# nnnagle/vq-vae

Measured on AMD Instinct MI355X. Metric: tiles/sec, higher is better.
Workload: dtype bf16

## Files before the change

### vq-vae_amd/csrc/enc_fused.hip

```cpp
#include "frl_common.hpp"
#include "frl_host.hpp"
#include "frl_pack.hpp"
#include "frl_reduce.hpp"

typedef bf16 TT;
typedef bf16x8 frag8;
#define EF_C0 64
#define EF_C1 128
#define EF_C2 64
#define EF_G 8
#define EF_NW 8
#define EF_NTH (64 * EF_NW)
#define EF_W1_FRAGS (8 * 2 * 64)
#define EF_W2_FRAGS (4 * 4 * 64)
#define EF_W2T_FRAGS (8 * 2 * 64)
#define EF_SLAB 384

template <int CTRL> __device__ __forceinline__ float ef_dpp(float v) {
  return __builtin_bit_cast(float, __builtin_amdgcn_update_dpp(0, __builtin_bit_cast(int, v), CTRL, 0xf, 0xf, true));
}
__device__ __forceinline__ float ef_row_sum(float v) {
  v += ef_dpp<0xB1>(v);
  v += ef_dpp<0x4E>(v);
  v += ef_dpp<0x124>(v);
// ... 187 lines not shown
    }
    bf16x8* zo = reinterpret_cast<bf16x8*>(zb + (int64_t)(t * 16 + px) * EF_C2 + 16 * kc);
    zo[0] = o0;
    zo[1] = o1;
    xt = xn;
  }
}

template <int NCH>
__device__ __forceinline__ void ef_channel_totals(const float (&p0)[NCH], const float (&p1)[NCH], float* __restrict__ part, float* __restrict__ chan,
                                                  float* __restrict__ out0, float* __restrict__ out1, int tid) {
  constexpr int C = 4 * NCH;
  const int lane = tid & 63, wave = tid >> 6, px = lane & 15, kc = lane >> 4;
#pragma unroll
  for (int j = 0; j < NCH; ++j) {
    const float a = ef_row_sum(p0[j]), q = ef_row_sum(p1[j]);
    if (px == 0) { part[(wave * 2 + 0) * C + NCH * kc + j] = a; part[(wave * 2 + 1) * C + NCH * kc + j] = q; }
  }
  __syncthreads();
  for (int i = tid; i < 2 * C; i += EF_NTH) {
    const int which = i / C, c = i % C;
    float s = 0.f;
    for (int w = 0; w < EF_NW; ++w) s += part[(w * 2 + which) * C + c];
    chan[which * C + c] = s;
    (which == 0 ? out0 : out1)[c] = s;
  }
  __syncthreads();
}

#define EF_PA 72
#define EF_PB 136
#define EF_OFF_TA (EF_OFF_TAB + EF_T_END * 4)
#define EF_OFF_TB (EF_OFF_TA + 128 * EF_PA * 2)
#define EF_LDS_BWD (EF_OFF_TB + 128 * EF_PB * 2)
#define EF_SLAB2 (EF_C2 * EF_C1 + EF_C1 * EF_C0 + EF_SLAB)

__device__ __forceinline__ bf16x8 ef_tr_frag(const TT* tile, int pitch, int pix0, int ch0, int r16) {
  const TT* a0 = tile + (pix0 + (r16 >> 2)) * pitch + ch0 + 4 * (r16 & 3);
  const bf16x4 lo = __builtin_amdgcn_ds_read_tr16_b64_v4bf16((bf16x4 __attribute__((address_space(3)))*)(a0));
  const bf16x4 hi = __builtin_amdgcn_ds_read_tr16_b64_v4bf16((bf16x4 __attribute__((address_space(3)))*)(a0 + 4 * pitch));
  return bf16x8{lo[0], lo[1], lo[2], lo[3], hi[0], hi[1], hi[2], hi[3]};
}
template <int NF>
__device__ __forceinline__ void ef_tile_put(TT* tile, int pitch, int prow, int kc, const LQTile<TT, NF>& t) {
  bf16x8* p = reinterpret_cast<bf16x8*>(tile + prow * pitch + NF * 8 * kc);
#pragma unroll
  for (int s = 0; s < NF; ++s) p[s] = t.f[s];
}

__global__ __launch_bounds__(EF_NTH) void enc2_bwd_kernel(const TT* __restrict__ X, const TT* __restrict__ DZ, const frag8* __restrict__ Wpk,
                                                          const float* __restrict__ g1, const float* __restrict__ b1,
                                                          const float* __restrict__ g2, const float* __restrict__ b2,
                                                          const float* __restrict__ stats, float* __restrict__ slab, int HW) {
  extern __shared__ __attribute__((aligned(16))) char smem[];
  const frag8* w1 = reinterpret_cast<const frag8*>(smem);
  const frag8* w2 = reinterpret_cast<const frag8*>(smem + EF_OFF_W2);
  const frag8* w2t = reinterpret_cast<const frag8*>(smem + EF_OFF_W2T);
  float* tab = reinterpret_cast<float*>(smem + EF_OFF_TAB);
  float* chan = tab + EF_T_CH;
  float* part = chan + 4 * 128;
  TT* tA = reinterpret_cast<TT*>(smem + EF_OFF_TA);
  TT* tB = reinterpret_cast<TT*>(smem + EF_OFF_TB);
  const int tid = threadIdx.x, lane = tid & 63, wave = tid >> 6, px = lane & 15, kc = lane >> 4;
  const int b = blockIdx.x;
  const TT* xb = X + (int64_t)b * HW * EF_C0;
  const TT* dzb = DZ + (int64_t)b * HW * EF_C2;
  float* my = slab + (int64_t)b * EF_SLAB2;
  float* myg = my + EF_C2 * EF_C1 + EF_C1 * EF_C0;
  copy_frags_lds<TT>(reinterpret_cast<frag8*>(smem), Wpk, EF_W1_FRAGS + EF_W2_FRAGS + EF_W2T_FRAGS, tid, EF_NTH);
  if (tid < 32) tab[EF_T_ST1 + tid] = stats[(int64_t)b * 32 + tid];
  __syncthreads();
  for (int c = tid; c < EF_C1 + EF_C2; c += EF_NTH) {
    if (c < EF_C1) {
      const float a = tab[EF_T_ST1 + 8 + c / 16] * g1[c];
      tab[EF_T_A1 + c] = a;
      tab[EF_T_O1 + c] = fmaf(-tab[EF_T_ST1 + c / 16], a, b1[c]);
    } else {
      const int c2 = c - EF_C1;
      const float a = tab[EF_T_ST2 + 8 + c2 / 8] * g2[c2];
      tab[EF_T_A2 + c2] = a;
      tab[EF_T_O2 + c2] = fmaf(-tab[EF_T_ST2 + c2 / 8], a, b2[c2]);
    }
  }
  __syncthreads();
  const int ntile = HW >> 4;
  const int nround = (ntile + EF_NW - 1) / EF_NW;
  const float* a1q = tab + EF_T_A1 + 32 * kc;
  const float* o1q = tab + EF_T_O1 + 32 * kc;
  const float* a2q = tab + EF_T_A2 + 16 * kc;
  const float mu2[2] = {tab[EF_T_ST2 + 2 * kc], tab[EF_T_ST2 + 2 * kc + 1]}, rs2[2] = {tab[EF_T_ST2 + 8 + 2 * kc], tab[EF_T_ST2 + 8 + 2 * kc + 1]};
  const float mu1[2] = {tab[EF_T_ST1 + 2 * kc], tab[EF_T_ST1 + 2 * kc + 1]}, rs1[2] = {tab[EF_T_ST1 + 8 + 2 * kc], tab[EF_T_ST1 + 8 + 2 * kc + 1]};

  auto chain = [&](const LQTile<TT, 2>& xt, float (&y1)[32], LQTile<TT, 4>& ht, float (&y2)[16], int lw) {
    ef_conv1(y1, xt, w1, lw);
#pragma unroll
    for (int j = 0; j < 32; ++j) {
      float v = fmaf(y1[j], a1q[j], o1q[j]);
      v = v > 0.f ? v : 0.f;
      ht.f[j >> 3][j & 7] = (bf16)v;
    }
    ef_conv2(y2, ht, w2, lw);
  };

  {
    float p0[16], p1[16];
#pragma unroll
    for (int j = 0; j < 16; ++j) { p0[j] = 0.f; p1[j] = 0.f; }
    for (int t = wave; t < ntile; t += EF_NW) {
      int lw = lane;
      asm volatile("" : "+v"(lw));
      LQTile<TT, 2> xt, dt;
      lq_load<TT, 2>(xt, xb, t * 16 + px, EF_C0, kc, true);
      lq_load<TT, 2>(dt, dzb, t * 16 + px, EF_C2, kc, true);
      float y1[32], y2[16];
      LQTile<TT, 4> ht;
      chain(xt, y1, ht, y2, lw);
#pragma unroll
      for (int j = 0; j < 16; ++j) {
        const float d = (float)dt.f[j >> 3][j & 7];
        const float xh = (y2[j] - mu2[j >> 3]) * rs2[j >> 3];
        p0[j] += d;
        p1[j] = fmaf(d, xh, p1[j]);
      }
    }
    ef_channel_totals<16>(p0, p1, part, chan, myg, myg + 64, tid);
  }
  float e2[2], f2[2];
  {
    const float inv_n = 1.f / ((float)(EF_C2 / EF_G) * (float)HW);
#pragma unroll
    for (int g = 0; g < 2; ++g) {
      float S1 = 0.f, S2 = 0.f;
      for (int c = (2 * kc + g) * 8; c < (2 * kc + g + 1) * 8; ++c) { S1 = fmaf(g2[c], chan[c], S1); S2 = fmaf(g2[c], chan[64 + c], S2); }
      e2[g] = -rs2[g] * rs2[g] * S2 * inv_n;
      f2[g] = -rs2[g] * S1 * inv_n - e2[g] * mu2[g];
    }
  }
  __syncthreads();

  auto back2 = [&](const LQTile<TT, 2>& dt, const float (&y1)[32], const float (&y2)[16], LQTile<TT, 2>& gt, float (&d1)[32], int lw) {
#pragma unroll
    for (int j = 0; j < 16; ++j) {
      const float d = (float)dt.f[j >> 3][j & 7];
      gt.f[j >> 3][j & 7] = (bf16)fmaf(a2q[j], d, fmaf(e2[j >> 3], y2[j], f2[j >> 3]));
    }
#pragma unroll
    for (int m = 0; m < 8; ++m) {
      f32x4 a = f32x4{0.f, 0.f, 0.f, 0.f};
#pragma unroll
      for (int s = 0; s < 2; ++s) a = mfma16(w2t[(m * 2 + s) * 64 + lw], gt.f[s], a);
#pragma unroll
      for (int r = 0; r < 4; ++r) {
        const int j = 4 * m + r;
        float v = ef_r(a[r]);
        if (!(fmaf(y1[j], a1q[j], o1q[j]) > 0.f)) v = 0.f;
        d1[j] = v;
      }
    }
  };

  const int ob2 = wave & 3, ig2 = wave >> 2;
  {
    f32x4 acc2[4];
#pragma unroll
    for (int i = 0; i < 4; ++i) acc2[i] = f32x4{0.f, 0.f, 0.f, 0.f};
    float p0[32], p1[32];
#pragma unroll
    for (int j = 0; j < 32; ++j) { p0[j] = 0.f; p1[j] = 0.f; }
    for (int r = 0; r < nround; ++r) {
      const int t = r * EF_NW + wave;
      const bool valid = t < ntile;
      int lw = lane;
      asm volatile("" : "+v"(lw));
      LQTile<TT, 2> gt;
      LQTile<TT, 4> ht;
      if (valid) {
        LQTile<TT, 2> xt, dt;
        lq_load<TT, 2>(xt, xb, t * 16 + px, EF_C0, kc, true);
        lq_load<TT, 2>(dt, dzb, t * 16 + px, EF_C2, kc, true);
        float y1[32], y2[16], d1[32];
        chain(xt, y1, ht, y2, lw);
        back2(dt, y1, y2, gt, d1, lw);
#pragma unroll
        for (int j = 0; j < 32; ++j) {
          const float xh = (y1[j] - mu1[j >> 4]) * rs1[j >> 4];
          p0[j] += d1[j];
          p1[j] = fmaf(d1[j], xh, p1[j]);
        }
      } else {
#pragma unroll
        for (int s = 0; s < 2; ++s) gt.f[s] = frag8{};
#pragma unroll
        for (int s = 0; s < 4; ++s) ht.f[s] = frag8{};
      }
      ef_tile_put<2>(tA, EF_PA, wave * 16 + px, kc, gt);
      ef_tile_put<4>(tB, EF_PB, wave * 16 + px, kc, ht);
      __syncthreads();
#pragma unroll
      for (int ks = 0; ks < 4; ++ks) {
        const bf16x8 af = ef_tr_frag(tA, EF_PA, 32 * ks + 8 * kc, 16 * ob2, px);
#pragma unroll
        for (int i = 0; i < 4; ++i) acc2[i] = mfma16(af, ef_tr_frag(tB, EF_PB, 32 * ks + 8 * kc, 16 * (4 * ig2 + i), px), acc2[i]);
      }
      __syncthreads();
    }
#pragma unroll
    for (int i = 0; i < 4; ++i)
#pragma unroll
      for (int rr = 0; rr < 4; ++rr) my[(16 * ob2 + 4 * kc + rr) * EF_C1 + 16 * (4 * ig2 + i) + px] = acc2[i][rr];
    ef_channel_totals<32>(p0, p1, part, chan, myg + 128, myg + 256, tid);
  }
  float e1[2], f1[2];
  {
    const float inv_n = 1.f / ((float)(EF_C1 / EF_G) * (float)HW);
#pragma unroll
    for (int g = 0; g < 2; ++g) {
      float S1 = 0.f, S2 = 0.f;
      for (int c = (2 * kc + g) * 16; c < (2 * kc + g + 1) * 16; ++c) { S1 = fmaf(g1[c], chan[c], S1); S2 = fmaf(g1[c], chan[128 + c], S2); }
      e1[g] = -rs1[g] * rs1[g] * S2 * inv_n;
      f1[g] = -rs1[g] * S1 * inv_n - e1[g] * mu1[g];
    }
  }
  {
    f32x4 acc1[4];
#pragma unroll
    for (int i = 0; i < 4; ++i) acc1[i] = f32x4{0.f, 0.f, 0.f, 0.f};
    float* my1 = my + EF_C2 * EF_C1;
    for (int r = 0; r < nround; ++r) {
      const int t = r * EF_NW + wave;
      const bool valid = t < ntile;
      int lw = lane;
      asm volatile("" : "+v"(lw));
      LQTile<TT, 2> xt;
      LQTile<TT, 4> yt;
      if (valid) {
        LQTile<TT, 2> dt, gt;
        lq_load<TT, 2>(xt, xb, t * 16 + px, EF_C0, kc, true);
        lq_load<TT, 2>(dt, dzb, t * 16 + px, EF_C2, kc, true);
        float y1[32], y2[16], d1[32];
        LQTile<TT, 4> ht;
        chain(xt, y1, ht, y2, lw);
        back2(dt, y1, y2, gt, d1, lw);
#pragma unroll
        for (int j = 0; j < 32; ++j) yt.f[j >> 3][j & 7] = (bf16)fmaf(a1q[j], d1[j], fmaf(e1[j >> 4], y1[j], f1[j >> 4]));
      } else {
#pragma unroll
        for (int s = 0; s < 2; ++s) xt.f[s] = frag8{};
#pragma unroll
        for (int s = 0; s < 4; ++s) yt.f[s] = frag8{};
      }
      ef_tile_put<2>(tA, EF_PA, wave * 16 + px, kc, xt);
      ef_tile_put<4>(tB, EF_PB, wave * 16 + px, kc, yt);
      __syncthreads();
#pragma unroll
      for (int ks = 0; ks < 4; ++ks) {
        const bf16x8 af = ef_tr_frag(tB, EF_PB, 32 * ks + 8 * kc, 16 * wave, px);
#pragma unroll
        for (int i = 0; i < 4; ++i) acc1[i] = mfma16(af, ef_tr_frag(tA, EF_PA, 32 * ks + 8 * kc, 16 * i, px), acc1[i]);
      }
      __syncthreads();
    }
#pragma unroll
    for (int i = 0; i < 4; ++i)
#pragma unroll
      for (int rr = 0; rr < 4; ++rr) my1[(16 * wave + 4 * kc + rr) * EF_C0 + 16 * i + px] = acc1[i][rr];
  }
}


static const frag8* enc_packed(const float* w1, const float* w2, int bwd, frag8* ws_pk, hipStream_t st) {
  FrlPackJob jobs[3];
  size_t off = 0;
  jobs[0] = frl_pack_job_pw(w1, off, FRL_BF16, 2, EF_C1, EF_C0, 8, EF_C0, 1);
  off += (size_t)EF_W1_FRAGS * sizeof(frag8);
  jobs[1] = frl_pack_job_pw(w2, off, FRL_BF16, 4, EF_C2, EF_C1, 4, EF_C1, 1);
  off += (size_t)EF_W2_FRAGS * sizeof(frag8);
  int n = 2;
  if (bwd) {
    jobs[2] = frl_pack_job_pw(w2, off, FRL_BF16, 2, EF_C1, EF_C2, 8, 1, EF_C1);
    off += (size_t)EF_W2T_FRAGS * sizeof(frag8);
    n = 3;
  }
  bool hit = false;
  frag8* pk = ws_pk;
  if (void* img = frl_pack_cached(jobs, n, off, &hit)) pk = (frag8*)img;
  if (!hit) {
    FRL_LAUNCH((pack_weights_kernel<TT, 2>), dim3(4), dim3(256), 0, st, pk, w1, EF_C1, EF_C0, 8, (int64_t)EF_C0, (int64_t)1);
    FRL_LAUNCH((pack_weights_kernel<TT, 4>), dim3(4), dim3(256), 0, st, pk + EF_W1_FRAGS, w2, EF_C2, EF_C1, 4, (int64_t)EF_C1, (int64_t)1);
    if (bwd) FRL_LAUNCH((pack_weights_kernel<TT, 2>), dim3(4), dim3(256), 0, st, pk + EF_W1_FRAGS + EF_W2_FRAGS, w2, EF_C1, EF_C2, 8, (int64_t)1, (int64_t)EF_C1);
  }
  return pk;
}

extern "C" {

int frl_encoder2_supported(int C0, int C1, int C2, int G1, int G2, int HW, int dtype) {
  return (dtype == FRL_BF16 && C0 == EF_C0 && C1 == EF_C1 && C2 == EF_C2 && G1 == EF_G && G2 == EF_G && HW > 0 && (HW % 16) == 0) ? 1 : 0;
}

size_t frl_encoder2_workspace_bytes(int B) {
  return ((size_t)B * EF_SLAB2 * sizeof(float) + 255) / 256 * 256 + (size_t)(EF_W1_FRAGS + EF_W2_FRAGS + EF_W2T_FRAGS) * sizeof(frag8);
}

int frl_encoder2_fwd(const void* x, const float* w1, const float* g1, const float* b1, const float* w2, const float* g2, const float* b2,
                     void* z, float* stats, int B, int HW, float eps, void* ws, size_t ws_bytes, hipStream_t stream) {
  if (B <= 0 || HW <= 0 || (HW % 16) != 0) return frl_fail(-2, "encoder2_fwd: need B > 0 and HW a positive multiple of 16");
  if (ws_bytes < frl_encoder2_workspace_bytes(B)) return frl_fail(-4, "encoder2_fwd: workspace too small");
  char* wsb = (char*)ws;
  const frag8* pk = enc_packed(w1, w2, 0, reinterpret_cast<frag8*>(wsb + ((size_t)B * EF_SLAB2 * sizeof(float) + 255) / 256 * 256), stream);
  auto kern = enc2_fwd_kernel;
  FRL_HIP(hipFuncSetAttribute((const void*)kern, hipFuncAttributeMaxDynamicSharedMemorySize, (int)EF_LDS));
  FRL_LAUNCH(enc2_fwd_kernel, dim3(B), dim3(EF_NTH), EF_LDS, stream, (const TT*)x, pk, g1, b1, g2, b2, (TT*)z, stats, HW, eps);
  return frl_check_launch("encoder2_fwd");
}

int frl_encoder2_bwd(const void* x, const void* dz, const float* w1, const float* g1, const float* b1, const float* w2, const float* g2,
                     const float* b2, const float* stats, float* dw1, float* dg1, float* db1, float* dw2, float* dg2, float* db2,
                     int B, int HW, void* ws, size_t ws_bytes, hipStream_t stream) {
  if (B <= 0 || HW <= 0 || (HW % 16) != 0) return frl_fail(-2, "encoder2_bwd: need B > 0 and HW a positive multiple of 16");
  if (ws_bytes < frl_encoder2_workspace_bytes(B)) return frl_fail(-4, "encoder2_bwd: workspace too small");
  char* wsb = (char*)ws;
  const frag8* pk = enc_packed(w1, w2, 1, reinterpret_cast<frag8*>(wsb + ((size_t)B * EF_SLAB2 * sizeof(float) + 255) / 256 * 256), stream);
  auto kern = enc2_bwd_kernel;
  FRL_HIP(hipFuncSetAttribute((const void*)kern, hipFuncAttributeMaxDynamicSharedMemorySize, (int)EF_LDS_BWD));
  FRL_LAUNCH(enc2_bwd_kernel, dim3(B), dim3(EF_NTH), EF_LDS_BWD, stream, (const TT*)x, (const TT*)dz, pk, g1, b1, g2, b2, stats, (float*)ws, HW);
  launch_slab_reduce_deferrable<float, EncEpi>((const float*)ws, B, (int64_t)EF_SLAB2, EncEpi{dw2, dw1, db2, dg2, db1, dg1}, stream);
  return frl_check_launch("encoder2_bwd");
}

}
```

### include/frl_hip.h

```cpp
#ifndef FRL_HIP_H
#define FRL_HIP_H

#include <stddef.h>
#include <stdint.h>

#ifdef __cplusplus
extern "C" {
#endif

typedef void* frl_stream_t;

enum { FRL_F32 = 0, FRL_BF16 = 1, FRL_F16 = 2  };
enum { FRL_ACT_NONE = 0, FRL_ACT_RELU = 1, FRL_ACT_SIGMOID = 2 };

int frl_version(void);
const char* frl_last_error(void);
int frl_device_arch(char* buf, int n);
int frl_kernel_timing_enable(int on);
int frl_kernel_timing_report(char* buf, int n);

size_t frl_pack_cache_table_bytes(void);
int frl_pack_cache_create(void* arena, size_t bytes);
int frl_pack_cache_destroy(int handle);
int frl_pack_cache_activate(int handle);
int frl_pack_cache_images(int handle);
int frl_pack_cache_refresh(int handle, frl_stream_t stream);

size_t frl_conv_workspace_bytes(int Cin, int Cout, int taps);
int frl_conv1x1_fwd(const void* x, const float* w, const float* bias, void* y, int64_t P, int Cin, int Cout, int act,
                    int dtype, void* ws, size_t ws_bytes, frl_stream_t stream);
int frl_conv1x1_bwd_data(const void* dy, const void* y, int act, const float* w, void* dx, int64_t P, int Cin, int Cout,
                         int dtype, void* ws, size_t ws_bytes, frl_stream_t stream);
int frl_conv1x1_bwd_data_add(const void* dy, const void* y, int act, const float* w, void* dx, const void* add, int64_t P,
                             int Cin, int Cout, int dtype, void* ws, size_t ws_bytes, frl_stream_t stream);
int frl_wgrad_set_max_workgroups(int n);
size_t frl_conv1x1_bwd_weight_workspace_bytes(int64_t P, int Cin, int Cout);
int frl_conv1x1_bwd_weight(const void* dy, const void* y, int act, const void* x, float* dw, float* dbias, int64_t P,
                           int Cin, int Cout, int dtype, void* ws, size_t ws_bytes, frl_stream_t stream);
int frl_conv_tap_bwd_weight(const void* dy, const void* y, int act, const void* x, float* dw, int64_t dso, int64_t dsi,
                            float* dbias, int64_t P, int Cin, int Cout, int HW, int T, int toff, int dtype, void* ws,
                            size_t ws_bytes, int flags, frl_stream_t stream);

int frl_conv3x3_fwd(const void* x, const float* w, const float* bias, void* y, int B, int H, int W, int Cin, int Cout,
                    int act, int dtype, void* ws, size_t ws_bytes, frl_stream_t stream);
int frl_conv3x3_fwd_gate_blend(const void* x, const float* w, const float* bias, const void* smoothed, const void* residual, void* gate,
                               void* out, int B, int H, int W, int Cin, int Cout, int dtype, void* ws, size_t ws_bytes,
                               frl_stream_t stream);
int frl_conv3x3_bwd_data(const void* dy, const void* y, int act, const float* w, void* dx, int B, int H, int W, int Cin,
                         int Cout, int dtype, void* ws, size_t ws_bytes, frl_stream_t stream);
int frl_conv3x3_bwd_data_fused(const void* dy, const void* y, int act, const float* w, void* dx, const void* add,
                               const void* sub_from, void* out2, int B, int H, int W, int Cin, int Cout, int dtype, void* ws,
                               size_t ws_bytes, frl_stream_t stream);
int frl_conv3x3_bwd_data_outmask(const void* dy, const void* y, int act, const float* w, void* dx, const void* out_y, int out_act, int B,
                                 int H, int W, int Cin, int Cout, int dtype, void* ws, size_t ws_bytes, frl_stream_t stream);
size_t frl_conv3x3_bwd_weight_workspace_bytes(int B, int H, int W, int Cin, int Cout);
int frl_conv3x3_bwd_weight(const void* dy, const void* y, int act, const void* x, float* dw, float* dbias, int B, int H,
                           int W, int Cin, int Cout, int dtype, void* ws, size_t ws_bytes, int flags, frl_stream_t stream);
int frl_conv3x3_wgrad_force_generic(int on);
int frl_conv3x3_tile32(int on);

int frl_groupnorm_fwd(const void* x, const float* gamma, const float* beta, void* y, float* mean, float* rstd, int B,
                      int HW, int C, int G, float eps, int relu, int dtype, frl_stream_t stream);
size_t frl_groupnorm_bwd_workspace_bytes(int B, int C, int G);
int frl_groupnorm_bwd(const void* dy, const void* x, const float* gamma, const float* beta, const float* mean,
                      const float* rstd, void* dx, float* dgamma, float* dbeta, int B, int HW, int C, int G, int relu,
                      int dtype, void* ws, size_t ws_bytes, frl_stream_t stream);

int frl_scalar_combine(const float* const* terms_host, const float* coef_host, int n, float* out, float* ok_out, frl_stream_t stream);
// ... 258 lines not shown
```

### vq-vae_amd/csrc/pw_wgrad.hip

```cpp
#include "frl_common.hpp"
#include "frl_host.hpp"
#include "frl_reduce.hpp"
#include <type_traits>

#define WG_KP 64

template <typename T, int OBW, int IB>
__global__ __launch_bounds__(256) void pw_wgrad_kernel(
    const T* __restrict__ dY, const T* __restrict__ Ymask, int mask_act, const T* __restrict__ X,
    float* __restrict__ slab, int64_t P, int Cout, int Cin, int64_t rows_per_wg, int HW, int Tn, int toff,
    int use_tr, int64_t ldy) {
  typedef typename DT<T>::frag_t frag_t;
  typedef typename std::conditional<sizeof(T) == 2, bf16x8, f32x4>::type vec_t;
  constexpr int FE = DT<T>::FE;
  constexpr int VEC = DT<T>::VEC;
  extern __shared__ __attribute__((aligned(16))) char smem[];
  constexpr int CoP = OBW * 4 * 16, CiP = IB * 16;
  constexpr int pitchA = CoP + 8, pitchB = CiP + 8;
  constexpr int VPRA = CoP / VEC, VPRB = CiP / VEC;
  constexpr int NA = (WG_KP * VPRA + 255) / 256, NB = (WG_KP * VPRB + 255) / 256;
  T* ldsA = reinterpret_cast<T*>(smem);
  T* ldsB = ldsA + WG_KP * pitchA;
  const int tid = threadIdx.x, lane = tid & 63, wave = tid >> 6;
  const int r16 = lane & 15, kc = lane >> 4;
// ... 214 lines not shown
  if (lds > 64 * 1024) FRL_HIP(hipFuncSetAttribute((const void*)kern, hipFuncAttributeMaxDynamicSharedMemorySize, (int)lds));
  FRL_LAUNCH_AS("pw_wgrad_kernel", kern, dim3(nwg), dim3(256), lds, st, (const T*)dy, (const T*)ymask, mask_act, (const T*)x, ws,
                     P, Cout, Cin, rows, HW, Tn, toff, use_tr, ldy);
  return frl_check_launch("pw_wgrad");
}

template <typename T>
static int dispatch_wgrad(const void* dy, const void* ymask, int mask_act, const void* x, float* ws, int64_t P,
                          int Cout, int Cin, int HW, int Tn, int toff, int use_tr, int64_t ldy, hipStream_t st) {
  const int ob = (Cout + 63) / 64;
  const int ib = (Cin + 15) / 16;
#define WG_CASE(O, I) return launch_wgrad<T, O, I>(dy, ymask, mask_act, x, ws, P, Cout, Cin, HW, Tn, toff, use_tr, ldy, st)
  if (ob <= 1) {
    if (ib <= 1) WG_CASE(1, 1);
    if (ib <= 2) WG_CASE(1, 2);
    if (ib <= 4) WG_CASE(1, 4);
    if (ib <= 8) WG_CASE(1, 8);
    if (ib <= 16) WG_CASE(1, 16);
  } else if (ob <= 2) {
    if (ib <= 1) WG_CASE(2, 1);
    if (ib <= 2) WG_CASE(2, 2);
    if (ib <= 4) WG_CASE(2, 4);
    if (ib <= 8) WG_CASE(2, 8);
  } else if (ob <= 4) {
    if (ib <= 1) WG_CASE(4, 1);
    if (ib <= 2) WG_CASE(4, 2);
    if (ib <= 4) WG_CASE(4, 4);
    if (ib <= 8) WG_CASE(4, 8);
  }
#undef WG_CASE
  return frl_fail(-2, "conv1x1_bwd_weight: unsupported (Cout, Cin) combination");
}

extern "C" {

int frl_wgrad_set_max_workgroups(int n) {
  const int was = g_wgrad_max_wgs;
  if (n >= 64 && n <= 4096) g_wgrad_max_wgs = n;
  return was;
}

size_t frl_conv1x1_bwd_weight_workspace_bytes(int64_t P, int Cin, int Cout) {
  return (size_t)wgrad_nwg(P) * ((size_t)Cout * Cin + Cout) * sizeof(float);
}

static int conv_tap_bwd_weight(const void* dy, const void* y, int act, const void* x, float* dw, int64_t dso,
                               int64_t dsi, float* dbias, int64_t P, int Cin, int Cout, int HW, int T, int toff,
                               int dtype, void* ws, size_t ws_bytes, int flags, hipStream_t stream, bool may_defer) {
  if (P <= 0) return frl_fail(-2, "bwd_weight: empty input");
  if (ws_bytes < frl_conv1x1_bwd_weight_workspace_bytes(P, Cin, Cout)) return frl_fail(-4, "bwd_weight: workspace too small");
  const void* ym = act != FRL_ACT_NONE ? y : nullptr;
  const int use_tr = (flags & 1) ? 0 : 1;
  const size_t esz = dtype == FRL_BF16 ? 2 : 4;
  for (int oc0 = 0; oc0 < Cout; oc0 += 256) {
    const int co = (Cout - oc0) < 256 ? (Cout - oc0) : 256;
    const char* dyp = (const char*)dy + (size_t)oc0 * esz;
    const char* ymp = ym ? (const char*)ym + (size_t)oc0 * esz : nullptr;
    int rc;
    if (dtype == FRL_F32) rc = dispatch_wgrad<float>(dyp, ymp, act, x, (float*)ws, P, co, Cin, HW, T, toff, 0, Cout, stream);
    else if (dtype == FRL_BF16) rc = dispatch_wgrad<bf16>(dyp, ymp, act, x, (float*)ws, P, co, Cin, HW, T, toff, use_tr, Cout, stream);
    else return frl_fail(-2, "bwd_weight: bad dtype");
    if (rc) return rc;
    const int64_t n = (int64_t)co * Cin + co;
    launch_slab_reduce_deferrable<float, WgradEpi>((const float*)ws, wgrad_nwg(P), n,
                                        WgradEpi{dw + (int64_t)oc0 * dso, dso, dsi, dbias ? dbias + oc0 : nullptr, co, Cin, (flags & 2) ? 1 : 0}, stream,
                                        may_defer && Cout <= 256 && (flags & 2) == 0);
  }
  return frl_check_launch("slab_reduce");
}

int frl_conv_tap_bwd_weight(const void* dy, const void* y, int act, const void* x, float* dw, int64_t dso,
                            int64_t dsi, float* dbias, int64_t P, int Cin, int Cout, int HW, int T, int toff,
                            int dtype, void* ws, size_t ws_bytes, int flags, hipStream_t stream) {
  const bool plain = dso == Cin && dsi == 1 && T == 1 && toff == 0;
  return conv_tap_bwd_weight(dy, y, act, x, dw, dso, dsi, dbias, P, Cin, Cout, HW, T, toff, dtype, ws, ws_bytes, flags, stream, plain);
}

int frl_conv1x1_bwd_weight(const void* dy, const void* y, int act, const void* x, float* dw, float* dbias,
                           int64_t P, int Cin, int Cout, int dtype, void* ws, size_t ws_bytes, hipStream_t stream) {
  return conv_tap_bwd_weight(dy, y, act, x, dw, Cin, 1, dbias, P, Cin, Cout, 1, 1, 0, dtype, ws, ws_bytes, 0, stream, true);
}

}
```

### vq-vae_amd/frl_hip/_lib.py

```python
from __future__ import annotations

import ctypes
import os
from ctypes import c_char_p, c_float, c_int, c_int64, c_size_t, c_void_p

_HERE = os.path.dirname(os.path.abspath(__file__))
LIB_PATH = os.path.join(_HERE, "libfrlhip_%s.so" % os.environ["FRL_HIP_LIB_TAG"] if os.environ.get("FRL_HIP_LIB_TAG") else "libfrlhip.so")

F32, BF16, F16 = 0, 1, 2
ACT_NONE, ACT_RELU, ACT_SIGMOID = 0, 1, 2

_lib = None


class FrlHipError(RuntimeError):
    pass


P, I, L, F, S, D = c_void_p, c_int, c_int64, c_float, c_size_t, ctypes.c_double
SIGNATURES = {
    "frl_version": (c_int, []),
    "frl_last_error": (c_char_p, []),
    "frl_device_arch": (c_int, [c_char_p, I]),
    "frl_kernel_timing_enable": (c_int, [I]),
    "frl_kernel_timing_report": (c_int, [c_char_p, I]),
    "frl_pack_cache_table_bytes": (S, []),
    "frl_pack_cache_create": (c_int, [P, S]),
    "frl_pack_cache_destroy": (c_int, [I]),
    "frl_pack_cache_activate": (c_int, [I]),
    "frl_pack_cache_images": (c_int, [I]),
    "frl_pack_cache_refresh": (c_int, [I, P]),
    "frl_conv_workspace_bytes": (S, [I, I, I]),
    "frl_conv1x1_fwd": (c_int, [P, P, P, P, L, I, I, I, I, P, S, P]),
    "frl_conv1x1_bwd_data": (c_int, [P, P, I, P, P, L, I, I, I, P, S, P]),
    "frl_conv1x1_bwd_data_add": (c_int, [P, P, I, P, P, P, L, I, I, I, P, S, P]),
    "frl_wgrad_set_max_workgroups": (c_int, [I]),
    "frl_conv3x3_wgrad_force_generic": (c_int, [I]),
    "frl_conv3x3_tile32": (c_int, [I]),
    "frl_conv1x1_bwd_weight_workspace_bytes": (S, [L, I, I]),
    "frl_conv1x1_bwd_weight": (c_int, [P, P, I, P, P, P, L, I, I, I, P, S, P]),
    "frl_conv_tap_bwd_weight": (c_int, [P, P, I, P, P, L, L, P, L, I, I, I, I, I, I, P, S, I, P]),
    "frl_vq_workspace_bytes": (S, [L, I, I]),
    "frl_vq_assign_fwd": (c_int, [P, P, L, I, I, P, P, P, P, I, P, S, P]),
    "frl_vq_prepared_bytes": (S, [I, I]),
    "frl_vq_prepare": (c_int, [P, L, I, I, I, P, S, P]),
    "frl_vq_stream_tiles": (c_int, [I]),
    "frl_vq_assign_fwd_prepared": (c_int, [P, P, P, L, I, I, P, P, P, P, I, P, S, P]),
    "frl_vq_bwd": (c_int, [P, P, P, P, P, P, P, F, L, I, I, P, P, P, I, P, S, P]),
    "frl_vq_ema_update": (c_int, [P, P, I, I, F, F, P, P, P, P, P]),
    "frl_vq_revive_dead_codes": (c_int, [P, P, L, P, L, I, I, ctypes.c_uint64, P, P, P, I, P]),
    "frl_groupnorm_fwd": (c_int, [P, P, P, P, P, P, I, I, I, I, F, I, I, P]),
    "frl_groupnorm_bwd_workspace_bytes": (S, [I, I, I]),
    "frl_groupnorm_bwd": (c_int, [P, P, P, P, P, P, P, P, P, I, I, I, I, I, I, P, S, P]),
    "frl_scalar_combine": (c_int, [P, P, I, P, P, P]),
    "frl_scalar_fanout": (c_int, [P, P, I, P, P]),
    "frl_scalar_combine_dev": (c_int, [P, P, P, I, P, P, P]),
    "frl_scalar_combine_aux": (c_int, [P, P, P, P, I, P, P, P, P]),
    "frl_scalar_fanout_dev": (c_int, [P, P, P, I, P, P]),
    "frl_scalar_fanout_guard": (c_int, [P, P, P, P, I, P, P, P]),
    "frl_encoder2_supported": (c_int, [I, I, I, I, I, I, I]),
    "frl_encoder2_workspace_bytes": (S, [I]),
    "frl_encoder2_fwd": (c_int, [P, P, P, P, P, P, P, P, P, I, I, F, P, S, P]),
    "frl_encoder2_bwd": (c_int, [P, P, P, P, P, P, P, P, P, P, P, P, P, P, P, I, I, P, S, P]),
    "frl_decoder_mse_fused_supported": (c_int, [I, I, I, I]),
    "frl_decoder_mse_workspace_bytes": (S, [L, I]),
    "frl_decoder_mse_fwd": (c_int, [P, P, P, P, P, P, P, P, P, L, I, P, S, P]),
    "frl_decoder_mse_bwd": (c_int, [P, P, P, P, P, P, P, P, P, P, P, P, P, P, L, I, P, S, P]),
    "frl_decoder_mse_onepass_bytes": (S, [L, I]),
    "frl_decoder_mse_fwd_bwd": (c_int, [P, P, P, P, P, P, P, P, P, P, P, S, P, P, L, I, P]),
# ... 123 lines not shown
```

### vq-vae_amd/frl_hip/ops.py

```python
from __future__ import annotations

import ctypes
from typing import Optional, Tuple

import torch

from . import _lib
from ._lib import ACT_NONE, ACT_RELU, ACT_SIGMOID, BF16, F32, check

_WS = {}

_TIMING = {"on": False, "events": {}}


def set_timing(on: bool) -> None:
    _TIMING["on"] = bool(on)
    _TIMING["events"] = {}


def timing_summary():
    torch.cuda.synchronize()
    return {k: (len(v), sum(a.elapsed_time(b) for a, b in v)) for k, v in _TIMING["events"].items()}


# ... 249 lines not shown
    w = _f32(w.reshape(cout, cin), "w")
    dx = torch.empty(dy.shape[:-1] + (cin,), dtype=dy.dtype, device=dy.device)
    p = dy.numel() // cout
    lib = _lib.load()
    ws = workspace(lib.frl_conv_workspace_bytes(cin, cout, 1), dy.device)
    if add is not None:
        _chk_like(add, dx, "conv1x1_bwd_data.add")
        check(lib.frl_conv1x1_bwd_data_add(_p(dy), _p(y), act, _p(w), _p(dx), _p(add), p, cin, cout, _dt(dy), _p(ws), ws.numel(),
                                           _stream()), "frl_conv1x1_bwd_data_add")
        return dx
    check(lib.frl_conv1x1_bwd_data(_p(dy), _p(y), act, _p(w), _p(dx), p, cin, cout, _dt(dy), _p(ws), ws.numel(), _stream()),
          "frl_conv1x1_bwd_data")
    return dx


def _conv1x1_bwd_weight_impl(dy: torch.Tensor, x: torch.Tensor, y: Optional[torch.Tensor] = None, act: int = ACT_NONE,
                       want_bias: bool = True, scalar_frags: bool = False) -> Tuple[torch.Tensor, Optional[torch.Tensor]]:
    cout, cin = dy.shape[-1], x.shape[-1]
    _chk_rows(dy, cout, "bwd_weight.dy")
    _chk_rows(x, cin, "bwd_weight.x")
    p = dy.numel() // cout
    lib = _lib.load()
    nbytes = lib.frl_conv1x1_bwd_weight_workspace_bytes(p, cin, cout)
    ws = workspace(nbytes, dy.device)
    dw = grad_empty((cout, cin), dy.device)
    db = grad_empty((cout,), dy.device) if want_bias else None
    check(lib.frl_conv_tap_bwd_weight(_p(dy), _p(y), act, _p(x), _p(dw), cin, 1, _p(db), p, cin, cout, 1, 1, 0,
                                      _dt(dy), _p(ws), ws.numel(), 1 if scalar_frags else 0, _stream()),
          "frl_conv_tap_bwd_weight")
    return dw, db


conv1x1_bwd_weight = _timed("conv1x1_bwd_weight")(_conv1x1_bwd_weight_impl)


def vq_stream_tiles(nt: int) -> int:
    return int(_lib.load().frl_vq_stream_tiles(int(nt)))


@_timed("vq_prepare")
def vq_prepare(codebook: torch.Tensor, n_rows: int, dtype: torch.dtype, out: Optional[torch.Tensor] = None) -> torch.Tensor:
    k, d = codebook.shape
    cb = _f32(codebook, "codebook")
    lib = _lib.load()
    nbytes = lib.frl_vq_prepared_bytes(k, d)
    if out is None or out.numel() < nbytes or out.device != cb.device:
        out = torch.empty(nbytes, dtype=torch.uint8, device=cb.device)
    check(lib.frl_vq_prepare(_p(cb), int(n_rows), k, d, BF16 if dtype == torch.bfloat16 else F32, _p(out), out.numel(), _stream()),
          "frl_vq_prepare")
    return out


@_timed("vq_assign")
def vq_assign(z: torch.Tensor, codebook: torch.Tensor, prep: Optional[torch.Tensor] = None):
    k, d = codebook.shape
    _chk_rows(z, d, "vq_assign.z")
    cb = _f32(codebook, "codebook")
    n = z.numel() // d
    lib = _lib.load()
    ws = workspace(lib.frl_vq_workspace_bytes(n, k, d), z.device)
    idx = torch.empty(n, dtype=torch.int32, device=z.device)
    zq = torch.empty_like(z)
    stats = torch.empty(4, dtype=torch.float32, device=z.device)
    counts = torch.empty(k, dtype=torch.int32, device=z.device)
    if prep is not None and (prep.dtype != torch.uint8 or prep.device != z.device or prep.numel() < lib.frl_vq_prepared_bytes(k, d)):
        raise ValueError("vq_assign: prep is not a prepared-codebook image for this codebook")
# ... 1388 lines not shown
```

Before: 109,000.

## Prefetch next tile rows into LDS via async global_load_lds in encoder backward

Result: no change. 109,200 (median of 6 runs) (+0.2%).

```diff
diff --git a/vq-vae_amd/csrc/enc_fused.hip b/vq-vae_amd/csrc/enc_fused.hip
--- a/vq-vae_amd/csrc/enc_fused.hip
+++ b/vq-vae_amd/csrc/enc_fused.hip
@@ -243,7 +243,15 @@
 #define EF_PB 136
 #define EF_OFF_TA (EF_OFF_TAB + EF_T_END * 4)
 #define EF_OFF_TB (EF_OFF_TA + 128 * EF_PA * 2)
-#define EF_LDS_BWD (EF_OFF_TB + 128 * EF_PB * 2)
+#define EF_OFF_ROWS (EF_OFF_TB + 128 * EF_PB * 2)
+#define EF_ROW_SEG 4096
+#define EF_OFF_GAM (EF_OFF_ROWS + EF_NW * EF_ROW_SEG)
+#define EF_LDS_BWD (EF_OFF_GAM + (EF_C1 + EF_C2) * 4)
+#ifdef EF_STAMPS
+#define EF_LDS_BWD_LAUNCH (EF_LDS_BWD + 1024)
+#else
+#define EF_LDS_BWD_LAUNCH EF_LDS_BWD
+#endif
 #define EF_SLAB2 (EF_C2 * EF_C1 + EF_C1 * EF_C0 + EF_SLAB)
 
 __device__ __forceinline__ bf16x8 ef_tr_frag(const TT* tile, int pitch, int pix0, int ch0, int r16) {
@@ -252,12 +260,33 @@
   const bf16x4 hi = __builtin_amdgcn_ds_read_tr16_b64_v4bf16((bf16x4 __attribute__((address_space(3)))*)(a0 + 4 * pitch));
   return bf16x8{lo[0], lo[1], lo[2], lo[3], hi[0], hi[1], hi[2], hi[3]};
 }
+__device__ __forceinline__ int ef_swz(int r) {
+  return ((r >> 1) & 1) | ((((r >> 1) ^ (r >> 2)) & 1) << 1) | (((r ^ (r >> 2) ^ (r >> 3)) & 1) << 2);
+}
+__device__ __forceinline__ void ef_dma_piece(const TT* base, unsigned voff, int ldst) {
+  unsigned keep;
+  asm volatile("s_mov_b32 %0, m0\n\ts_mov_b32 m0, %3\n\ts_nop 0\n\tglobal_load_lds_dwordx4 %1, %2\n\ts_mov_b32 m0, %0"
+               : "=&s"(keep) : "v"(voff), "s"(base), "s"(ldst) : "memory");
+}
 template <int NF>
 __device__ __forceinline__ void ef_tile_put(TT* tile, int pitch, int prow, int kc, const LQTile<TT, NF>& t) {
   bf16x8* p = reinterpret_cast<bf16x8*>(tile + prow * pitch + NF * 8 * kc);
 #pragma unroll
   for (int s = 0; s < NF; ++s) p[s] = t.f[s];
 }
+
+#ifndef EF_ROW_DMA
+#define EF_ROW_DMA 1
+#endif
+#ifdef EF_STAMPS
+__device__ unsigned long long* ef_dbg;
+#define EF_NST 16
+#define EF_ST(i) do { const unsigned long long t_now = __builtin_amdgcn_s_memtime(); if ((threadIdx.x & 63u) == 0) ef_ts[wv * EF_NST + (i)] += t_now - t_prev; t_prev = t_now; } while (0)
+#define EF_ST_DRAIN() asm volatile("s_waitcnt vmcnt(0) lgkmcnt(0)" ::: "memory")
+#else
+#define EF_ST(i) do { } while (0)
+#define EF_ST_DRAIN() do { } while (0)
+#endif
 
 __global__ __launch_bounds__(EF_NTH) void enc2_bwd_kernel(const TT* __restrict__ X, const TT* __restrict__ DZ, const frag8* __restrict__ Wpk,
                                                           const float* __restrict__ g1, const float* __restrict__ b1,
@@ -278,23 +307,80 @@
   const TT* dzb = DZ + (int64_t)b * HW * EF_C2;
   float* my = slab + (int64_t)b * EF_SLAB2;
   float* myg = my + EF_C2 * EF_C1 + EF_C1 * EF_C0;
+  const int ntile = HW >> 4;
+#ifdef EF_STAMPS
+  unsigned long long* ef_ts = reinterpret_cast<unsigned long long*>(smem + EF_LDS_BWD);
+  if (tid < EF_NW * EF_NST) ef_ts[tid] = 0ull;
+  __syncthreads();
+  unsigned long long t_prev = __builtin_amdgcn_s_memtime();
+  const unsigned long long t_start = t_prev, r_start = __builtin_amdgcn_s_memrealtime();
+#endif
+  const int wv = __builtin_amdgcn_readfirstlane(wave);
+  const int seg = EF_OFF_ROWS + wv * EF_ROW_SEG;
+  const unsigned rowpk = (unsigned)((lane >> 3) * 128 + (((lane & 7) ^ ef_swz(lane >> 3)) << 4)) |
+                         ((unsigned)(px * 128 + (((2 * kc) ^ ef_swz(px)) << 4)) << 16);
+  auto rows_request = [&](int t) {
+#if EF_ROW_DMA
+    unsigned k_ = rowpk;
+    asm volatile("" : "+v"(k_));
+    const unsigned v0 = k_ & 0xffffu, v1 = (v0 ^ 64u) + 1024u;
+    const int t0 = __builtin_amdgcn_readfirstlane(t);
+    const TT* xs = xb + (int64_t)t0 * (16 * EF_C0);
+    const TT* ds = dzb + (int64_t)t0 * (16 * EF_C2);
+    asm volatile("s_waitcnt lgkmcnt(0)" ::: "memory");
+    ef_dma_piece(xs, v0, seg);
+    ef_dma_piece(xs, v1, seg + 1024);
+    ef_dma_piece(ds, v0, seg + 2048);
+    ef_dma_piece(ds, v1, seg + 3072);
+#endif
+  };
+  auto rows_take = [&](LQTile<TT, 2>& xt, LQTile<TT, 2>& dt, int t) {
+#if !EF_ROW_DMA
+    lq_load<TT, 2>(xt, xb, t * 16 + px, EF_C0, kc, true);
+    lq_load<TT, 2>(dt, dzb, t * 16 + px, EF_C2, kc, true);
+#else
+    (void)t;
+    asm volatile("s_waitcnt vmcnt(0)" ::: "memory");
+    unsigned k_ = rowpk;
+    asm volatile("" : "+v"(k_));
+    const int f0 = seg + (int)(k_ >> 16), f1 = f0 ^ 16;
+    xt.f[0] = *reinterpret_cast<const frag8*>(smem + f0);
+    xt.f[1] = *reinterpret_cast<const frag8*>(smem + f1);
+    dt.f[0] = *reinterpret_cast<const frag8*>(smem + 2048 + f0);
+    dt.f[1] = *reinterpret_cast<const frag8*>(smem + 2048 + f1);
+#endif
+  };
+  if (wv < ntile) rows_request(wv);
+  EF_ST(15);
+  float* gam1 = reinterpret_cast<float*>(smem + EF_OFF_GAM);
+  float* gam2 = gam1 + EF_C1;
+  const float* sb = stats + (int64_t)b * 32;
+#if EF_ROW_DMA
+  {
+    unsigned l16 = (unsigned)lane * 16u;
+    asm volatile("" : "+v"(l16));
+#pragma unroll
+    for (int i = 0; i < (EF_W1_FRAGS + EF_W2_FRAGS + EF_W2T_FRAGS) / (64 * EF_NW); ++i)
+      ef_dma_piece(reinterpret_cast<const TT*>(Wpk) + (i * EF_NW + wv) * 512, l16, (i * EF_NW + wv) * 1024);
+  }
+#else
   copy_frags_lds<TT>(reinterpret_cast<frag8*>(smem), Wpk, EF_W1_FRAGS + EF_W2_FRAGS + EF_W2T_FRAGS, tid, EF_NTH);
-  if (tid < 32) tab[EF_T_ST1 + tid] = stats[(int64_t)b * 32 + tid];
-  __syncthreads();
-  for (int c = tid; c < EF_C1 + EF_C2; c += EF_NTH) {
-    if (c < EF_C1) {
-      const float a = tab[EF_T_ST1 + 8 + c / 16] * g1[c];
-      tab[EF_T_A1 + c] = a;
-      tab[EF_T_O1 + c] = fmaf(-tab[EF_T_ST1 + c / 16], a, b1[c]);
-    } else {
-      const int c2 = c - EF_C1;
-      const float a = tab[EF_T_ST2 + 8 + c2 / 8] * g2[c2];
-      tab[EF_T_A2 + c2] = a;
-      tab[EF_T_O2 + c2] = fmaf(-tab[EF_T_ST2 + c2 / 8], a, b2[c2]);
-    }
-  }
-  __syncthreads();
-  const int ntile = HW >> 4;
+#endif
+  {
+    const bool l1 = tid < EF_C1;
+    const int c = l1 ? tid : ((tid - EF_C1) & (EF_C2 - 1));
+    const int gi = l1 ? c / 16 : 16 + c / 8;
+    const float st = sb[tid & 31], g = (l1 ? g1 : g2)[c], bt = (l1 ? b1 : b2)[c], mu = sb[gi], rs = sb[8 + gi];
+    const float a = rs * g, o = fmaf(-mu, a, bt);
+    if (tid < 32) tab[EF_T_ST1 + tid] = st;
+    if (tid < EF_C1 + EF_C2) {
+      (l1 ? gam1 : gam2)[c] = g;
+      tab[(l1 ? EF_T_A1 : EF_T_A2) + c] = a;
+      tab[(l1 ? EF_T_O1 : EF_T_O2) + c] = o;
+    }
+  }
+  asm volatile("s_waitcnt vmcnt(0)" ::: "memory");
+  __syncthreads();
   const int nround = (ntile + EF_NW - 1) / EF_NW;
   const float* a1q = tab + EF_T_A1 + 32 * kc;
   const float* o1q = tab + EF_T_O1 + 32 * kc;
@@ -321,8 +407,12 @@
       int lw = lane;
       asm volatile("" : "+v"(lw));
       LQTile<TT, 2> xt, dt;
-      lq_load<TT, 2>(xt, xb, t * 16 + px, EF_C0, kc, true);
-      lq_load<TT, 2>(dt, dzb, t * 16 + px, EF_C2, kc, true);
+      EF_ST(15);
+      rows_take(xt, dt, t);
+      EF_ST_DRAIN();
+      EF_ST(0);
+      rows_request(t + EF_NW < ntile ? t + EF_NW : wv);
+      EF_ST(1);
       float y1[32], y2[16];
       LQTile<TT, 4> ht;
       chain(xt, y1, ht, y2, lw);
@@ -333,6 +423,7 @@
         p0[j] += d;
         p1[j] = fmaf(d, xh, p1[j]);
       }
+      EF_ST(2);
     }
     ef_channel_totals<16>(p0, p1, part, chan, myg, myg + 64, tid);
   }
@@ -342,7 +433,7 @@
 #pragma unroll
     for (int g = 0; g < 2; ++g) {
       float S1 = 0.f, S2 = 0.f;
-      for (int c = (2 * kc + g) * 8; c < (2 * kc + g + 1) * 8; ++c) { S1 = fmaf(g2[c], chan[c], S1); S2 = fmaf(g2[c], chan[64 + c], S2); }
+      for (int c = (2 * kc + g) * 8; c < (2 * kc + g + 1) * 8; ++c) { S1 = fmaf(gam2[c], chan[c], S1); S2 = fmaf(gam2[c], chan[64 + c], S2); }
       e2[g] = -rs2[g] * rs2[g] * S2 * inv_n;
       f2[g] = -rs2[g] * S1 * inv_n - e2[g] * mu2[g];
     }
@@ -387,8 +478,12 @@
       LQTile<TT, 4> ht;
       if (valid) {
         LQTile<TT, 2> xt, dt;
-        lq_load<TT, 2>(xt, xb, t * 16 + px, EF_C0, kc, true);
-        lq_load<TT, 2>(dt, dzb, t * 16 + px, EF_C2, kc, true);
+        EF_ST(15);
+        rows_take(xt, dt, t);
+        EF_ST_DRAIN();
+        EF_ST(3);
+        rows_request(t + EF_NW < ntile ? t + EF_NW : wv);
+        EF_ST(4);
         float y1[32], y2[16], d1[32];
         chain(xt, y1, ht, y2, lw);
         back2(dt, y1, y2, gt, d1, lw);
@@ -398,6 +493,7 @@
           p0[j] += d1[j];
           p1[j] = fmaf(d1[j], xh, p1[j]);
         }
+        EF_ST(5);
       } else {
 #pragma unroll
         for (int s = 0; s < 2; ++s) gt.f[s] = frag8{};
@@ -407,13 +503,16 @@
       ef_tile_put<2>(tA, EF_PA, wave * 16 + px, kc, gt);
       ef_tile_put<4>(tB, EF_PB, wave * 16 + px, kc, ht);
       __syncthreads();
+      EF_ST(6);
 #pragma unroll
       for (int ks = 0; ks < 4; ++ks) {
         const bf16x8 af = ef_tr_frag(tA, EF_PA, 32 * ks + 8 * kc, 16 * ob2, px);
 #pragma unroll
         for (int i = 0; i < 4; ++i) acc2[i] = mfma16(af, ef_tr_frag(tB, EF_PB, 32 * ks + 8 * kc, 16 * (4 * ig2 + i), px), acc2[i]);
       }
+      EF_ST(7);
       __syncthreads();
+      EF_ST(8);
     }
 #pragma unroll
     for (int i = 0; i < 4; ++i)
@@ -427,7 +526,7 @@
 #pragma unroll
     for (int g = 0; g < 2; ++g) {
       float S1 = 0.f, S2 = 0.f;
-      for (int c = (2 * kc + g) * 16; c < (2 * kc + g + 1) * 16; ++c) { S1 = fmaf(g1[c], chan[c], S1); S2 = fmaf(g1[c], chan[128 + c], S2); }
+      for (int c = (2 * kc + g) * 16; c < (2 * kc + g + 1) * 16; ++c) { S1 = fmaf(gam1[c], chan[c], S1); S2 = fmaf(gam1[c], chan[128 + c], S2); }
       e1[g] = -rs1[g] * rs1[g] * S2 * inv_n;
       f1[g] = -rs1[g] * S1 * inv_n - e1[g] * mu1[g];
     }
@@ -446,14 +545,19 @@
       LQTile<TT, 4> yt;
       if (valid) {
         LQTile<TT, 2> dt, gt;
-        lq_load<TT, 2>(xt, xb, t * 16 + px, EF_C0, kc, true);
-        lq_load<TT, 2>(dt, dzb, t * 16 + px, EF_C2, kc, true);
+        EF_ST(15);
+        rows_take(xt, dt, t);
+        EF_ST_DRAIN();
+        EF_ST(9);
+        if (t + EF_NW < ntile) rows_request(t + EF_NW);
+        EF_ST(10);
         float y1[32], y2[16], d1[32];
         LQTile<TT, 4> ht;
         chain(xt, y1, ht, y2, lw);
         back2(dt, y1, y2, gt, d1, lw);
 #pragma unroll
         for (int j = 0; j < 32; ++j) yt.f[j >> 3][j & 7] = (bf16)fmaf(a1q[j], d1[j], fmaf(e1[j >> 4], y1[j], f1[j >> 4]));
+        EF_ST(11);
       } else {
 #pragma unroll
         for (int s = 0; s < 2; ++s) xt.f[s] = frag8{};
@@ -463,19 +567,31 @@
       ef_tile_put<2>(tA, EF_PA, wave * 16 + px, kc, xt);
       ef_tile_put<4>(tB, EF_PB, wave * 16 + px, kc, yt);
       __syncthreads();
+      EF_ST(12);
 #pragma unroll
       for (int ks = 0; ks < 4; ++ks) {
         const bf16x8 af = ef_tr_frag(tB, EF_PB, 32 * ks + 8 * kc, 16 * wave, px);
 #pragma unroll
         for (int i = 0; i < 4; ++i) acc1[i] = mfma16(af, ef_tr_frag(tA, EF_PA, 32 * ks + 8 * kc, 16 * i, px), acc1[i]);
       }
+      EF_ST(13);
       __syncthreads();
+      EF_ST(14);
     }
 #pragma unroll
     for (int i = 0; i < 4; ++i)
 #pragma unroll
       for (int rr = 0; rr < 4; ++rr) my1[(16 * wave + 4 * kc + rr) * EF_C0 + 16 * i + px] = acc1[i][rr];
   }
+#ifdef EF_STAMPS
+  EF_ST(15);
+  __syncthreads();
+  if (tid < EF_NW * EF_NST) ef_dbg[(size_t)blockIdx.x * (EF_NW * EF_NST) + tid] = ef_ts[tid];
+  if (tid == 0) {
+    ef_dbg[(size_t)gridDim.x * (EF_NW * EF_NST) + 2 * blockIdx.x] = __builtin_amdgcn_s_memtime() - t_start;
+    ef_dbg[(size_t)gridDim.x * (EF_NW * EF_NST) + 2 * blockIdx.x + 1] = __builtin_amdgcn_s_memrealtime() - r_start;
+  }
+#endif
 }
 
 
@@ -533,8 +649,8 @@
   char* wsb = (char*)ws;
   const frag8* pk = enc_packed(w1, w2, 1, reinterpret_cast<frag8*>(wsb + ((size_t)B * EF_SLAB2 * sizeof(float) + 255) / 256 * 256), stream);
   auto kern = enc2_bwd_kernel;
-  FRL_HIP(hipFuncSetAttribute((const void*)kern, hipFuncAttributeMaxDynamicSharedMemorySize, (int)EF_LDS_BWD));
-  FRL_LAUNCH(enc2_bwd_kernel, dim3(B), dim3(EF_NTH), EF_LDS_BWD, stream, (const TT*)x, (const TT*)dz, pk, g1, b1, g2, b2, stats, (float*)ws, HW);
+  FRL_HIP(hipFuncSetAttribute((const void*)kern, hipFuncAttributeMaxDynamicSharedMemorySize, (int)EF_LDS_BWD_LAUNCH));
+  FRL_LAUNCH(enc2_bwd_kernel, dim3(B), dim3(EF_NTH), EF_LDS_BWD_LAUNCH, stream, (const TT*)x, (const TT*)dz, pk, g1, b1, g2, b2, stats, (float*)ws, HW);
   launch_slab_reduce_deferrable<float, EncEpi>((const float*)ws, B, (int64_t)EF_SLAB2, EncEpi{dw2, dw1, db2, dg2, db1, dg1}, stream);
   return frl_check_launch("encoder2_bwd");
 }
```

## Add specialized thin-Cout pointwise weight-gradient kernel with async LDS prefetch ring

Applied to the files above, without the earlier changes.

After: 113,200 before, 114,400 after, median of 6. +1.1%, better.

```diff
diff --git a/include/frl_hip.h b/include/frl_hip.h
--- a/include/frl_hip.h
+++ b/include/frl_hip.h
@@ -34,6 +34,7 @@
 int frl_conv1x1_bwd_data_add(const void* dy, const void* y, int act, const float* w, void* dx, const void* add, int64_t P,
                              int Cin, int Cout, int dtype, void* ws, size_t ws_bytes, frl_stream_t stream);
 int frl_wgrad_set_max_workgroups(int n);
+int frl_wgrad_thin(int on);
 size_t frl_conv1x1_bwd_weight_workspace_bytes(int64_t P, int Cin, int Cout);
 int frl_conv1x1_bwd_weight(const void* dy, const void* y, int act, const void* x, float* dw, float* dbias, int64_t P,
                            int Cin, int Cout, int dtype, void* ws, size_t ws_bytes, frl_stream_t stream);
diff --git a/vq-vae_amd/csrc/pw_wgrad.hip b/vq-vae_amd/csrc/pw_wgrad.hip
--- a/vq-vae_amd/csrc/pw_wgrad.hip
+++ b/vq-vae_amd/csrc/pw_wgrad.hip
@@ -270,6 +270,10 @@
   return frl_fail(-2, "conv1x1_bwd_weight: unsupported (Cout, Cin) combination");
 }
 
+bool pwt_supported(const void* dy, const void* ymask, const void* x, int64_t P, int Cin, int Cout, int64_t ldy, int T, int toff, int dtype,
+                   int flags);
+int pwt_launch(const void* dy, const void* x, float* ws, int64_t P, int Cout, int nwg, int64_t rows, hipStream_t st);
+
 extern "C" {
 
 int frl_wgrad_set_max_workgroups(int n) {
@@ -295,7 +299,11 @@
     const char* dyp = (const char*)dy + (size_t)oc0 * esz;
     const char* ymp = ym ? (const char*)ym + (size_t)oc0 * esz : nullptr;
     int rc;
-    if (dtype == FRL_F32) rc = dispatch_wgrad<float>(dyp, ymp, act, x, (float*)ws, P, co, Cin, HW, T, toff, 0, Cout, stream);
+    if (pwt_supported(dyp, ymp, x, P, Cin, co, Cout, T, toff, dtype, flags)) {
+      const int nwg = wgrad_nwg(P);
+      const int64_t rows = ((P + nwg - 1) / nwg + WG_KP - 1) / WG_KP * WG_KP;
+      rc = pwt_launch(dyp, x, (float*)ws, P, co, nwg, rows, stream);
+    } else if (dtype == FRL_F32) rc = dispatch_wgrad<float>(dyp, ymp, act, x, (float*)ws, P, co, Cin, HW, T, toff, 0, Cout, stream);
     else if (dtype == FRL_BF16) rc = dispatch_wgrad<bf16>(dyp, ymp, act, x, (float*)ws, P, co, Cin, HW, T, toff, use_tr, Cout, stream);
     else return frl_fail(-2, "bwd_weight: bad dtype");
     if (rc) return rc;
diff --git a/vq-vae_amd/csrc/pw_wgrad_thin.hip b/vq-vae_amd/csrc/pw_wgrad_thin.hip
--- /dev/null
+++ b/vq-vae_amd/csrc/pw_wgrad_thin.hip
@@ -0,0 +1,169 @@
+#include "frl_common.hpp"
+#include "frl_host.hpp"
+
+#define PWT_KP 64
+#ifndef PWT_D
+#define PWT_D 4
+#endif
+#define PWT_XB (PWT_KP * 128)
+#define PWT_YB 2048
+#define PWT_SLOT (PWT_XB + PWT_YB)
+#define PWT_LDS (PWT_D * PWT_SLOT)
+
+__device__ __forceinline__ void pwt_glds16(const void* src, int lds_byte) {
+  unsigned keep;
+  asm volatile("s_mov_b32 %0, m0\n\ts_mov_b32 m0, %2\n\ts_nop 0\n\tglobal_load_lds_dwordx4 %1, off nt\n\ts_mov_b32 m0, %0"
+               : "=&s"(keep) : "v"(src), "s"(lds_byte) : "memory");
+}
+template <int N> __device__ __forceinline__ void pwt_vmcnt() { asm volatile("s_waitcnt vmcnt(%0)" ::"n"(N) : "memory"); }
+template <int K> __device__ __forceinline__ void pwt_wait(int rem) {
+  static_assert(PWT_D >= 3 && PWT_D - 2 <= 6 && 6 * K <= 63, "extend the chain below with the ring");
+  if (rem >= 6) pwt_vmcnt<6 * K>();
+  else if (rem == 5) pwt_vmcnt<5 * K>();
+  else if (rem == 4) pwt_vmcnt<4 * K>();
+  else if (rem == 3) pwt_vmcnt<3 * K>();
+  else if (rem == 2) pwt_vmcnt<2 * K>();
+  else if (rem == 1) pwt_vmcnt<K>();
+  else pwt_vmcnt<0>();
+}
+__device__ __forceinline__ bf16x8 pwt_tr8(const char* smem, int lo, int hi) {
+  const bf16x4 a = __builtin_amdgcn_ds_read_tr16_b64_v4bf16((bf16x4 __attribute__((address_space(3)))*)(smem + lo));
+  const bf16x4 b = __builtin_amdgcn_ds_read_tr16_b64_v4bf16((bf16x4 __attribute__((address_space(3)))*)(smem + hi));
+  return bf16x8{a[0], a[1], a[2], a[3], b[0], b[1], b[2], b[3]};
+}
+
+template <int COUT>
+__global__ __launch_bounds__(256) void pw_wgrad_thin_kernel(const bf16* __restrict__ dY, const bf16* __restrict__ X, float* __restrict__ slab,
+                                                            int64_t P, int64_t rows_per_wg) {
+  static_assert(COUT % 4 == 0 && COUT <= 16, "thin outputs only");
+  constexpr int NVY = PWT_KP * COUT / 8;
+  constexpr int NPY = (NVY + 63) / 64;
+  extern __shared__ __attribute__((aligned(16))) char smem[];
+  const int tid = threadIdx.x, lane = tid & 63;
+  const int wave = __builtin_amdgcn_readfirstlane(tid >> 6);
+  const int r16 = lane & 15, kc = lane >> 4;
+
+  const int64_t p_begin = (int64_t)blockIdx.x * rows_per_wg;
+  int64_t p_end = p_begin + rows_per_wg;
+  if (p_end > P) p_end = P;
+  const int nt = p_end > p_begin ? (int)((p_end - p_begin) / PWT_KP) : 0;
+
+  const int xr8 = lane >> 3, xc = lane & 7;
+  auto issue = [&](int i, int slot) {
+    const int64_t p0 = p_begin + (int64_t)i * PWT_KP;
+    const int base = slot * PWT_SLOT;
+#pragma unroll
+    for (int j = 0; j < 2; ++j) {
+      const int piece = 2 * wave + j;
+      const int f = ((xr8 >> 1) & 1) | ((piece & 1) << 1);
+      pwt_glds16(X + (p0 + piece * 8 + xr8) * 64 + ((xc ^ (f << 1)) << 3), base + piece * 1024);
+    }
+    if (wave < NPY) {
+      int v = wave * 64 + lane;
+      v = v < NVY ? v : NVY - 1;
+      pwt_glds16(dY + p0 * COUT + v * 8, base + PWT_XB + wave * 1024);
+    }
+  };
+  auto wait_oldest = [&](int rem) {
+    if (wave < NPY) pwt_wait<3>(rem);
+    else pwt_wait<2>(rem);
+  };
+
+  const int fr = ((r16 >> 3) & 1) | ((kc & 1) << 1);
+  const int xrow = (8 * kc + (r16 >> 2)) * 128 + ((r16 & 3) >> 1) * 16 + (r16 & 1) * 8;
+  int xoff[4];
+#pragma unroll
+  for (int i = 0; i < 4; ++i) xoff[i] = xrow + ((i ^ fr) << 5);
+  const int yoff = PWT_XB + ((8 * kc + (r16 >> 2)) * COUT + 4 * (r16 & 3)) * 2;
+  const bf16 one_ = (r16 == 0) ? (bf16)1.f : (bf16)0.f;
+  const bf16x8 ones = bf16x8{one_, one_, one_, one_, one_, one_, one_, one_};
+
+  f32x4 acc[4], accb = f32x4{0.f, 0.f, 0.f, 0.f};
+#pragma unroll
+  for (int i = 0; i < 4; ++i) acc[i] = f32x4{0.f, 0.f, 0.f, 0.f};
+
+  int issued = 0, islot = 0, cslot = 0;
+  for (; issued < PWT_D - 1 && issued < nt; ++issued) {
+    issue(issued, islot);
+    ++islot;
+  }
+  for (int t = 0; t < nt; ++t) {
+    wait_oldest(issued - 1 - t);
+    asm volatile("s_waitcnt lgkmcnt(0)" ::: "memory");
+    __builtin_amdgcn_s_barrier();
+    asm volatile("" ::: "memory");
+    if (issued < nt) {
+      issue(issued, islot);
+      ++issued;
+      islot = islot + 1 == PWT_D ? 0 : islot + 1;
+    }
+    if (wave == 0) {
+      const char* tb = smem + cslot * PWT_SLOT;
+#pragma unroll
+      for (int ks = 0; ks < PWT_KP / 32; ++ks) {
+        const bf16x8 af = pwt_tr8(tb, yoff + ks * (32 * COUT * 2), yoff + ks * (32 * COUT * 2) + 4 * COUT * 2);
+        bf16x8 bf[4];
+#pragma unroll
+        for (int i = 0; i < 4; ++i) bf[i] = pwt_tr8(tb, xoff[i] + ks * (32 * 128), xoff[i] + ks * (32 * 128) + 4 * 128);
+#pragma unroll
+        for (int i = 0; i < 4; ++i) acc[i] = mfma16(af, bf[i], acc[i]);
+        accb = mfma16(af, ones, accb);
+      }
+    }
+    cslot = cslot + 1 == PWT_D ? 0 : cslot + 1;
+  }
+
+  if (wave == 0) {
+    float* my = slab + (int64_t)blockIdx.x * (COUT * 64 + COUT);
+#pragma unroll
+    for (int i = 0; i < 4; ++i)
+#pragma unroll
+      for (int r = 0; r < 4; ++r) {
+        const int oc = kc * 4 + r;
+        if (oc < COUT) my[oc * 64 + i * 16 + r16] = acc[i][r];
+      }
+    if (r16 == 0) {
+#pragma unroll
+      for (int r = 0; r < 4; ++r) {
+        const int oc = kc * 4 + r;
+        if (oc < COUT) my[COUT * 64 + oc] = accb[r];
+      }
+    }
+  }
+}
+
+static int g_wgrad_thin = 1;
+
+bool pwt_supported(const void* dy, const void* ymask, const void* x, int64_t P, int Cin, int Cout, int64_t ldy, int T, int toff, int dtype,
+                   int flags) {
+  return g_wgrad_thin && dtype == FRL_BF16 && Cin == 64 && (Cout % 4) == 0 && Cout >= 4 && Cout <= 16 && ldy == Cout && ymask == nullptr &&
+         T == 1 && toff == 0 && P > 0 && (P % PWT_KP) == 0 && (flags & 1) == 0 && ((uintptr_t)dy % 16) == 0 && ((uintptr_t)x % 16) == 0;
+}
+
+template <int COUT>
+static void pwt_launch_t(const void* dy, const void* x, float* ws, int64_t P, int nwg, int64_t rows, hipStream_t st) {
+  if (PWT_LDS > 64 * 1024) (void)hipFuncSetAttribute((const void*)pw_wgrad_thin_kernel<COUT>, hipFuncAttributeMaxDynamicSharedMemorySize, PWT_LDS);
+  FRL_LAUNCH_AS("pw_wgrad_thin_kernel", pw_wgrad_thin_kernel<COUT>, dim3(nwg), dim3(256), PWT_LDS, st, (const bf16*)dy, (const bf16*)x, ws, P,
+                rows);
+}
+
+int pwt_launch(const void* dy, const void* x, float* ws, int64_t P, int Cout, int nwg, int64_t rows, hipStream_t st) {
+  switch (Cout) {
+    case 4: pwt_launch_t<4>(dy, x, ws, P, nwg, rows, st); break;
+    case 8: pwt_launch_t<8>(dy, x, ws, P, nwg, rows, st); break;
+    case 12: pwt_launch_t<12>(dy, x, ws, P, nwg, rows, st); break;
+    case 16: pwt_launch_t<16>(dy, x, ws, P, nwg, rows, st); break;
+    default: return frl_fail(-2, "pw_wgrad_thin: unsupported Cout");
+  }
+  return frl_check_launch("pw_wgrad_thin");
+}
+
+extern "C" {
+
+int frl_wgrad_thin(int on) {
+  const int was = g_wgrad_thin;
+  g_wgrad_thin = on ? 1 : 0;
+  return was;
+}
+
+}
diff --git a/vq-vae_amd/frl_hip/_lib.py b/vq-vae_amd/frl_hip/_lib.py
--- a/vq-vae_amd/frl_hip/_lib.py
+++ b/vq-vae_amd/frl_hip/_lib.py
@@ -35,6 +35,7 @@
     "frl_conv1x1_bwd_data": (c_int, [P, P, I, P, P, L, I, I, I, P, S, P]),
     "frl_conv1x1_bwd_data_add": (c_int, [P, P, I, P, P, P, L, I, I, I, P, S, P]),
     "frl_wgrad_set_max_workgroups": (c_int, [I]),
+    "frl_wgrad_thin": (c_int, [I]),
     "frl_conv3x3_wgrad_force_generic": (c_int, [I]),
     "frl_conv3x3_tile32": (c_int, [I]),
     "frl_conv1x1_bwd_weight_workspace_bytes": (S, [L, I, I]),
diff --git a/vq-vae_amd/frl_hip/ops.py b/vq-vae_amd/frl_hip/ops.py
--- a/vq-vae_amd/frl_hip/ops.py
+++ b/vq-vae_amd/frl_hip/ops.py
@@ -305,6 +305,10 @@
 
 
 conv1x1_bwd_weight = _timed("conv1x1_bwd_weight")(_conv1x1_bwd_weight_impl)
+
+
+def wgrad_thin(on: bool) -> bool:
+    return bool(_lib.load().frl_wgrad_thin(1 if on else 0))
 
 
 def vq_stream_tiles(nt: int) -> int:
```
